# EPFL-VILAB/MultiMAE

Hardware: NVIDIA H100
Metric: MultiMAE-B pretrain samples/sec @ bs=128/GPU (higher is better)
Workload: dtype bf16

## Files before the change

multimae_b200/csrc/common.cuh:

```cuda
#pragma once

#include <cuda.h>
#include <cuda_bf16.h>
#include <cuda_runtime.h>
#include <stdint.h>

namespace mmae {

typedef __nv_bfloat16 bf16;

void set_last_error(const char* fmt, ...);

#define MMAE_CHECK(cond, code, ...)                    \
  do {                                                 \
    if (!(cond)) {                                     \
      ::mmae::set_last_error(__VA_ARGS__);             \
      return (code);                                   \
    }                                                  \
  } while (0)

#define MMAE_CUDA_OK(expr)                                                               \
  do {                                                                                   \
    cudaError_t _e = (expr);                                                             \
    if (_e != cudaSuccess) {                                                             \
// ... 129 lines not shown

__device__ __forceinline__ uint4 ld_stream_16_rw(const void* p) {
  uint4 v;
  asm volatile("ld.global.L1::no_allocate.v4.u32 {%0, %1, %2, %3}, [%4];"
               : "=r"(v.x), "=r"(v.y), "=r"(v.z), "=r"(v.w)
               : "l"(p));
  return v;
}

__device__ __forceinline__ void mbar_init(uint64_t* bar, uint32_t count) {
  asm volatile("mbarrier.init.shared::cta.b64 [%0], %1;" ::"r"(smem_u32(bar)), "r"(count) : "memory");
}
__device__ __forceinline__ void fence_barrier_init() {
  asm volatile("fence.mbarrier_init.release.cluster;" ::: "memory");
}
__device__ __forceinline__ void fence_proxy_async_smem() {
  asm volatile("fence.proxy.async.shared::cta;" ::: "memory");
}
__device__ __forceinline__ void mbar_expect_tx(uint64_t* bar, uint32_t bytes) {
  asm volatile("mbarrier.arrive.expect_tx.shared::cta.b64 _, [%0], %1;" ::"r"(smem_u32(bar)), "r"(bytes)
               : "memory");
}
__device__ __forceinline__ void mbar_arrive(uint64_t* bar) {
  asm volatile("mbarrier.arrive.shared::cta.b64 _, [%0];" ::"r"(smem_u32(bar)) : "memory");
}
__device__ __forceinline__ bool mbar_try_wait(uint64_t* bar, uint32_t parity) {
  uint32_t ok;
  asm volatile(
      "{\n\t"
      ".reg .pred P1;\n\t"
      "mbarrier.try_wait.parity.shared::cta.b64 P1, [%1], %2;\n\t"
      "selp.u32 %0, 1, 0, P1;\n\t"
      "}\n"
      : "=r"(ok)
      : "r"(smem_u32(bar)), "r"(parity)
      : "memory");
  return ok != 0;
}
__device__ __forceinline__ void mbar_wait(uint64_t* bar, uint32_t parity) {
  while (!mbar_try_wait(bar, parity)) {
  }
}

__device__ __forceinline__ void tma_prefetch_desc(const CUtensorMap* m) {
  asm volatile("prefetch.tensormap [%0];" ::"l"(reinterpret_cast<uint64_t>(m)) : "memory");
}
__device__ __forceinline__ void tma_load_2d(void* smem_dst, const CUtensorMap* m, uint64_t* bar, int c0,
                                            int c1) {
  asm volatile(
      "cp.async.bulk.tensor.2d.shared::cluster.global.mbarrier::complete_tx::bytes [%0], [%1, {%3, %4}], [%2];"
      :
      : "r"(smem_u32(smem_dst)), "l"(reinterpret_cast<uint64_t>(m)), "r"(smem_u32(bar)), "r"(c0), "r"(c1)
      : "memory");
}
__device__ __forceinline__ void tma_load_2d_multicast(void* smem_dst, const CUtensorMap* m, uint64_t* bar, int c0, int c1,
                                                      uint16_t cta_mask) {
  asm volatile(
      "cp.async.bulk.tensor.2d.shared::cluster.global.mbarrier::complete_tx::bytes.multicast::cluster [%0], [%1, {%3, %4}], "
      "[%2], %5;"
      :
      : "r"(smem_u32(smem_dst)), "l"(reinterpret_cast<uint64_t>(m)), "r"(smem_u32(bar)), "r"(c0), "r"(c1), "h"(cta_mask)
      : "memory");
}
__device__ __forceinline__ void tma_store_2d(const CUtensorMap* m, const void* smem_src, int c0, int c1) {
  asm volatile("cp.async.bulk.tensor.2d.global.shared::cta.bulk_group [%0, {%2, %3}], [%1];"
               :
               : "l"(reinterpret_cast<uint64_t>(m)), "r"(smem_u32(smem_src)), "r"(c0), "r"(c1)
               : "memory");
}
__device__ __forceinline__ void tma_reduce_add_2d(const CUtensorMap* m, const void* smem_src, int c0, int c1) {
  asm volatile("cp.reduce.async.bulk.tensor.2d.global.shared::cta.add.tile.bulk_group [%0, {%2, %3}], [%1];"
               :
               : "l"(reinterpret_cast<uint64_t>(m)), "r"(smem_u32(smem_src)), "r"(c0), "r"(c1)
               : "memory");
}
__device__ __forceinline__ void tma_store_3d(const CUtensorMap* m, const void* smem_src, int c0, int c1, int c2) {
  asm volatile("cp.async.bulk.tensor.3d.global.shared::cta.bulk_group [%0, {%2, %3, %4}], [%1];"
               :
               : "l"(reinterpret_cast<uint64_t>(m)), "r"(smem_u32(smem_src)), "r"(c0), "r"(c1), "r"(c2)
               : "memory");
}
__device__ __forceinline__ void bulk_commit_group() { asm volatile("cp.async.bulk.commit_group;" ::: "memory"); }
__device__ __forceinline__ void bulk_wait_read_all() { asm volatile("cp.async.bulk.wait_group.read 0;" ::: "memory"); }
__device__ __forceinline__ void bulk_wait_all() { asm volatile("cp.async.bulk.wait_group 0;" ::: "memory"); }
__device__ __forceinline__ void tma_load_3d(void* smem_dst, const CUtensorMap* m, uint64_t* bar, int c0,
                                            int c1, int c2) {
  asm volatile(
      "cp.async.bulk.tensor.3d.shared::cluster.global.mbarrier::complete_tx::bytes [%0], [%1, {%3, %4, %5}], "
      "[%2];"
      :
      : "r"(smem_u32(smem_dst)), "l"(reinterpret_cast<uint64_t>(m)), "r"(smem_u32(bar)), "r"(c0), "r"(c1),
        "r"(c2)
      : "memory");
}

__device__ __forceinline__ uint32_t cluster_ctarank() {
  uint32_t r;
  asm volatile("mov.u32 %0, %%cluster_ctarank;" : "=r"(r));
  return r;
}
__device__ __forceinline__ void cluster_sync_all() {
  asm volatile("barrier.cluster.arrive.release.aligned;\n\tbarrier.cluster.wait.acquire.aligned;" ::: "memory");
}
__device__ __forceinline__ uint32_t mapa_u32(uint32_t smem_addr, uint32_t rank) {
  uint32_t r;
  asm volatile("mapa.shared::cluster.u32 %0, %1, %2;" : "=r"(r) : "r"(smem_addr), "r"(rank));
  return r;
}

__device__ __forceinline__ void wgmma_fence() { asm volatile("wgmma.fence.sync.aligned;" ::: "memory"); }
__device__ __forceinline__ void wgmma_commit() { asm volatile("wgmma.commit_group.sync.aligned;" ::: "memory"); }
template <int N>
__device__ __forceinline__ void wgmma_wait() {
  asm volatile("wgmma.wait_group.sync.aligned %0;" ::"n"(N) : "memory");
}
__device__ __forceinline__ void reg_fence(float& r) { asm volatile("" : "+f"(r)::"memory"); }

template <int R>
__device__ __forceinline__ void setmaxnreg_inc() {
  asm volatile("setmaxnreg.inc.sync.aligned.u32 %0;" ::"n"(R));
}
template <int R>
__device__ __forceinline__ void setmaxnreg_dec() {
  asm volatile("setmaxnreg.dec.sync.aligned.u32 %0;" ::"n"(R));
}

__device__ __forceinline__ uint64_t gmma_desc_sw128(uint32_t smem_addr, uint32_t lbo_bytes, uint32_t sbo_bytes) {
  uint64_t d = 0;
  d |= uint64_t((smem_addr & 0x3FFFFu) >> 4);
  d |= uint64_t((lbo_bytes >> 4) & 0x3FFFu) << 16;
  d |= uint64_t((sbo_bytes >> 4) & 0x3FFFu) << 32;
  d |= uint64_t(1) << 62;
  return d;
}

__device__ __forceinline__ void mbar_arrive_cluster(uint32_t mbar_cluster) {
  asm volatile("mbarrier.arrive.release.cluster.shared::cluster.b64 _, [%0];" ::"r"(mbar_cluster) : "memory");
}

__device__ __forceinline__ uint64_t gmma_desc_noswz(uint32_t smem_addr, uint32_t lbo_bytes, uint32_t sbo_bytes) {
  uint64_t d = 0;
  d |= uint64_t((smem_addr & 0x3FFFFu) >> 4);
  d |= uint64_t((lbo_bytes >> 4) & 0x3FFFu) << 16;
  d |= uint64_t((sbo_bytes >> 4) & 0x3FFFu) << 32;
  return d;
}

template <int TA, int TB>
__device__ __forceinline__ void wgmma_m64n64k16(float (&d)[32], uint64_t desc_a, uint64_t desc_b, uint32_t scale_d) {
  asm volatile(
      "{\n.reg .pred p;\nsetp.ne.b32 p, %34, 0;\n"
      "wgmma.mma_async.sync.aligned.m64n64k16.f32.bf16.bf16 "
      "{"
      "%0, %1, %2, %3, %4, %5, %6, %7, %8, %9, %10, %11, %12, %13, %14, %15, "
      "%16, %17, %18, %19, %20, %21, %22, %23, %24, %25, %26, %27, %28, %29, %30, %31"
      "}, %32, %33, p, 1, 1, %35, %36;\n}\n"
      : "+f"(d[0]), "+f"(d[1]), "+f"(d[2]), "+f"(d[3]), "+f"(d[4]), "+f"(d[5]), "+f"(d[6]), "+f"(d[7]),
        "+f"(d[8]), "+f"(d[9]), "+f"(d[10]), "+f"(d[11]), "+f"(d[12]), "+f"(d[13]), "+f"(d[14]), "+f"(d[15]),
        "+f"(d[16]), "+f"(d[17]), "+f"(d[18]), "+f"(d[19]), "+f"(d[20]), "+f"(d[21]), "+f"(d[22]), "+f"(d[23]),
        "+f"(d[24]), "+f"(d[25]), "+f"(d[26]), "+f"(d[27]), "+f"(d[28]), "+f"(d[29]), "+f"(d[30]), "+f"(d[31])
      : "l"(desc_a), "l"(desc_b), "r"(scale_d), "n"(TA), "n"(TB));
}
template <int TA, int TB>
__device__ __forceinline__ void wgmma_m64n192k16(float (&d)[96], uint64_t desc_a, uint64_t desc_b, uint32_t scale_d) {
  asm volatile(
      "{\n.reg .pred p;\nsetp.ne.b32 p, %98, 0;\n"
// ... 117 lines not shown
```

multimae_b200/csrc/gemm_wgmma.cu:

```cuda
#include <algorithm>
#include <cstdlib>

#include "common.cuh"
#include "../../include/multimae_b200.h"

namespace mmae {

void count_launch();
bool gemm_profile_begin(cudaStream_t st, double flops, int M, int N, int K, int flags);
void gemm_profile_end(cudaStream_t st);

namespace {

constexpr int BM = 128;
constexpr int BK = 64;
constexpr int WG_K = 16;
constexpr int GEMM_THREADS = 384;

struct GemmParams {
  int M, N, K;
  int num_kb;
  int kb_per_split;
  int tma_store;
  mmae_gemm_epilogue ep;
};

template <int BN>
struct GemmCfg {
  static constexpr int STAGES = BN == 256 ? 4 : (BN == 192 ? 5 : (BN == 128 ? 6 : 8));
  static constexpr int A_BYTES = BM * BK * 2;
  static constexpr int B_BYTES = BN * BK * 2;
  static constexpr int STAGE_BYTES = A_BYTES + B_BYTES;
  static constexpr int BAR_OFFSET = STAGES * STAGE_BYTES;
  static constexpr int TOTAL = BAR_OFFSET + 256 + 1024;
  static_assert(TOTAL <= 232448, "GEMM exceeds the 227 KB shared-memory limit");
};

__device__ __forceinline__ void red_add_v2(float* addr, float a, float b) {
  asm volatile("red.global.add.v2.f32 [%0], {%1, %2};" ::"l"(addr), "f"(a), "f"(b) : "memory");
}

__device__ __forceinline__ void epilogue_pair(float v0, float v1, int row, int n, const GemmParams& p, bool first_split,
                                              bool atomic_out) {
  const mmae_gemm_epilogue& ep = p.ep;
  v0 *= ep.alpha;
  v1 *= ep.alpha;
  if (ep.bias && first_split) {
    const float2 b = __ldg(reinterpret_cast<const float2*>(ep.bias + n));
    v0 += b.x;
    v1 += b.y;
  }
  if (ep.preact_bf16)
    *reinterpret_cast<uint32_t*>(reinterpret_cast<bf16*>(ep.preact_bf16) + int64_t(row) * ep.ld_preact + n) = pack_bf16x2(v0, v1);
  if (ep.act == 1) {
    v0 = gelu_erf(v0);
    v1 = gelu_erf(v1);
  }
  if (ep.dgelu_z) {
    const uint32_t z = __ldg(reinterpret_cast<const unsigned int*>(reinterpret_cast<const bf16*>(ep.dgelu_z) +
                                                                   int64_t(row) * ep.ld_dgelu_z + n));
    const float2 zf = unpack_bf16x2(z);
    v0 *= dgelu_erf(zf.x);
    v1 *= dgelu_erf(zf.y);
  }
  if (ep.residual && first_split) {
    const float2 r = __ldg(reinterpret_cast<const float2*>(ep.residual + int64_t(row) * ep.ld_residual + n));
    v0 += r.x;
    v1 += r.y;
  }
  if (ep.out_f32) {
    float* dst = ep.out_f32 + int64_t(row) * ep.ld_out_f32 + n;
    if (atomic_out) red_add_v2(dst, v0, v1);
    else *reinterpret_cast<float2*>(dst) = make_float2(v0, v1);
  }
  if (ep.out_bf16)
    *reinterpret_cast<uint32_t*>(reinterpret_cast<bf16*>(ep.out_bf16) + int64_t(row) * ep.ld_out_bf16 + n) = pack_bf16x2(v0, v1);
}

template <typename T>
__device__ __forceinline__ void stage_pair(uint8_t* stage, int r, int c, float v0, float v1) {
  T* box = reinterpret_cast<T*>(stage + (c >> 5) * (64 * 32 * sizeof(T)));
  if constexpr (sizeof(T) == 4) *reinterpret_cast<float2*>(box + r * 32 + (c & 31)) = make_float2(v0, v1);
  else *reinterpret_cast<uint32_t*>(box + r * 32 + (c & 31)) = pack_bf16x2(v0, v1);
}

template <int BN, int CL, bool A_MN, bool B_MN>
__global__ void __launch_bounds__(GEMM_THREADS, 1)
    gemm_bf16_kernel(const __grid_constant__ CUtensorMap tmA, const __grid_constant__ CUtensorMap tmB,
                     const __grid_constant__ CUtensorMap tmC, const GemmParams p) {
  pdl_launch_dependents();
  using C = GemmCfg<BN>;
  constexpr int STAGES = C::STAGES;
  constexpr int BH = BN / CL;
  static_assert(!B_MN || BH % 64 == 0, "MN-major B is loaded in 64-column chunks");

  extern __shared__ uint8_t smem_raw[];
  const uint32_t raw_addr = smem_u32(smem_raw);
  uint8_t* smem = smem_raw + ((1024u - (raw_addr & 1023u)) & 1023u);
  uint64_t* full_bar = reinterpret_cast<uint64_t*>(smem + C::BAR_OFFSET);
  uint64_t* empty_bar = full_bar + STAGES;

  const int wg = threadIdx.x >> 7;
  const int rank = CL > 1 ? int(cluster_ctarank()) : 0;
  const int n0 = blockIdx.x * BN;
  const int m0 = blockIdx.y * BM;
  const int kb_begin = blockIdx.z * p.kb_per_split;
  int nkb = p.num_kb - kb_begin;
  if (nkb > p.kb_per_split) nkb = p.kb_per_split;
  if (nkb < 0) nkb = 0;

  if (threadIdx.x == 0) {
    tma_prefetch_desc(&tmA);
    tma_prefetch_desc(&tmB);
    if (p.tma_store) tma_prefetch_desc(&tmC);
#pragma unroll
    for (int s = 0; s < STAGES; ++s) {
      mbar_init(&full_bar[s], 1);
      mbar_init(&empty_bar[s], 2 * CL);
    }
    fence_barrier_init();
  }
  __syncthreads();
  if constexpr (CL > 1) cluster_sync_all();
  pdl_wait();

  if (wg == 0) {
    setmaxnreg_dec<40>();
    if (threadIdx.x == 0) {
      for (int kb = 0; kb < nkb; ++kb) {
        const int s = kb % STAGES;
        const uint32_t ph = (kb / STAGES) & 1;
        mbar_wait(&empty_bar[s], ph ^ 1u);
        mbar_expect_tx(&full_bar[s], C::STAGE_BYTES);
        uint8_t* sA = smem + s * C::STAGE_BYTES;
        uint8_t* sB = sA + C::A_BYTES;
        const int k0 = (kb_begin + kb) * BK;
        if constexpr (!A_MN) {
          tma_load_2d(sA, &tmA, &full_bar[s], k0, m0);
        } else {
#pragma unroll
          for (int c = 0; c < BM / 64; ++c) tma_load_2d(sA + c * (64 * BK * 2), &tmA, &full_bar[s], m0 + c * 64, k0);
        }
        if constexpr (CL == 1) {
          if constexpr (!B_MN) {
            tma_load_2d(sB, &tmB, &full_bar[s], k0, n0);
          } else {
#pragma unroll
            for (int c = 0; c < BN / 64; ++c) tma_load_2d(sB + c * (64 * BK * 2), &tmB, &full_bar[s], n0 + c * 64, k0);
          }
        } else {
          if constexpr (!B_MN) {
            tma_load_2d_multicast(sB + rank * BH * 128, &tmB, &full_bar[s], k0, n0 + rank * BH, 0x3);
          } else {
#pragma unroll
            for (int c = 0; c < BH / 64; ++c)
              tma_load_2d_multicast(sB + (rank * (BH / 64) + c) * (64 * BK * 2), &tmB, &full_bar[s], n0 + rank * BH + c * 64,
                                    k0, 0x3);
          }
        }
      }
    }
  } else {
    setmaxnreg_inc<232>();
    const int cw = wg - 1;
    float acc[BN / 2];

    for (int kb = 0; kb < nkb; ++kb) {
      const int s = kb % STAGES;
      const uint32_t ph = (kb / STAGES) & 1;
      mbar_wait(&full_bar[s], ph);
      const uint32_t a_addr = smem_u32(smem + s * C::STAGE_BYTES) + cw * (64 * BK * 2);
      const uint32_t b_addr = smem_u32(smem + s * C::STAGE_BYTES) + C::A_BYTES;
#pragma unroll
      for (int i = 0; i < BN / 2; ++i) reg_fence(acc[i]);
      wgmma_fence();
#pragma unroll
      for (int j = 0; j < BK / WG_K; ++j) {
        const uint32_t sd = (kb | j) != 0 ? 1u : 0u;
        const uint64_t da = A_MN ? gmma_desc_sw128(a_addr + j * (WG_K * 128), 64 * BK * 2, 1024)
                                 : gmma_desc_sw128(a_addr + j * (WG_K * 2), 16, 1024);
        const uint64_t db = B_MN ? gmma_desc_sw128(b_addr + j * (WG_K * 128), 64 * BK * 2, 1024)
                                 : gmma_desc_sw128(b_addr + j * (WG_K * 2), 16, 1024);
        if constexpr (BN == 256) wgmma_m64n256k16<A_MN ? 1 : 0, B_MN ? 1 : 0>(acc, da, db, sd);
        else if constexpr (BN == 192) wgmma_m64n192k16<A_MN ? 1 : 0, B_MN ? 1 : 0>(acc, da, db, sd);
        else if constexpr (BN == 128) wgmma_m64n128k16<A_MN ? 1 : 0, B_MN ? 1 : 0>(acc, da, db, sd);
        else wgmma_m64n64k16<A_MN ? 1 : 0, B_MN ? 1 : 0>(acc, da, db, sd);
      }
      wgmma_commit();
#pragma unroll
      for (int i = 0; i < BN / 2; ++i) reg_fence(acc[i]);
      wgmma_wait<1>();
      if (kb > 0 && (threadIdx.x & 127) == 0) {
        const int rs = (kb - 1) % STAGES;
        if constexpr (CL == 1) mbar_arrive(&empty_bar[rs]);
        else
          for (int r = 0; r < CL; ++r) mbar_arrive_cluster(mapa_u32(smem_u32(&empty_bar[rs]), uint32_t(r)));
      }
    }
    wgmma_wait<0>();
#pragma unroll
    for (int i = 0; i < BN / 2; ++i) reg_fence(acc[i]);

    const int t = threadIdx.x & 127;
    const int rl = (t >> 5) * 16 + ((t & 31) >> 2);
    const int row_a = m0 + cw * 64 + rl;
    const int row_b = row_a + 8;
    const bool first_split = blockIdx.z == 0;
    if (nkb > 0 && p.tma_store) {
      asm volatile("bar.sync 1, 256;" ::: "memory");
      uint8_t* stage = smem + cw * (64 * BN * (p.tma_store == 1 ? 2 : 4));
      const float* bias = first_split ? p.ep.bias : nullptr;
#pragma unroll
      for (int j = 0; j < BN / 8; ++j) {
        const int c = j * 8 + 2 * (t & 3);
        float v[4] = {acc[4 * j] * p.ep.alpha, acc[4 * j + 1] * p.ep.alpha, acc[4 * j + 2] * p.ep.alpha,
                      acc[4 * j + 3] * p.ep.alpha};
        if (bias && n0 + c < p.N) {
          const float2 bb = __ldg(reinterpret_cast<const float2*>(bias + n0 + c));
          v[0] += bb.x; v[1] += bb.y; v[2] += bb.x; v[3] += bb.y;
        }
        if (p.ep.act == 1) {
#pragma unroll
          for (int i = 0; i < 4; ++i) v[i] = gelu_erf(v[i]);
        }
        if (p.tma_store == 1) {
          stage_pair<bf16>(stage, rl, c, v[0], v[1]);
          stage_pair<bf16>(stage, rl + 8, c, v[2], v[3]);
        } else {
          stage_pair<float>(stage, rl, c, v[0], v[1]);
          stage_pair<float>(stage, rl + 8, c, v[2], v[3]);
        }
      }
      fence_proxy_async_smem();
      asm volatile("bar.sync %0, 128;" ::"r"(2 + cw) : "memory");
      if (t == 0) {
        const int box_bytes = 64 * 32 * (p.tma_store == 1 ? 2 : 4);
        for (int b = 0; b < BN / 32 && n0 + b * 32 < p.N; ++b) {
          if (p.tma_store == 3) tma_reduce_add_2d(&tmC, stage + b * box_bytes, n0 + b * 32, m0 + cw * 64);
          else tma_store_2d(&tmC, stage + b * box_bytes, n0 + b * 32, m0 + cw * 64);
        }
        bulk_commit_group();
        bulk_wait_all();
      }
    } else if (nkb > 0) {
      const bool atomic_out = p.ep.accumulate != 0 || gridDim.z > 1;
#pragma unroll
      for (int j = 0; j < BN / 8; ++j) {
        if (n0 + j * 8 >= p.N) break;
        const int n = n0 + j * 8 + 2 * (t & 3);
        if (row_a < p.M) epilogue_pair(acc[4 * j], acc[4 * j + 1], row_a, n, p, first_split, atomic_out);
        if (row_b < p.M) epilogue_pair(acc[4 * j + 2], acc[4 * j + 3], row_b, n, p, first_split, atomic_out);
      }
    }
  }
  if constexpr (CL > 1) cluster_sync_all();
}

template <int BN, int CL, bool A_MN, bool B_MN>
int launch_gemm(const CUtensorMap& tmA, const CUtensorMap& tmB, const CUtensorMap& tmC, const GemmParams& p, int split_k,
                cudaStream_t stream) {
  using C = GemmCfg<BN>;
  auto kern = gemm_bf16_kernel<BN, CL, A_MN, B_MN>;
  static bool configured = false;
  if (!configured) {
    MMAE_CUDA_OK(cudaFuncSetAttribute(kern, cudaFuncAttributeMaxDynamicSharedMemorySize, C::TOTAL));
    configured = true;
  }
  dim3 grid(ceil_div(p.N, BN), ceil_div(ceil_div(p.M, BM), CL) * CL, split_k);
  const bool prof = gemm_profile_begin(stream, 2.0 * p.M * p.N * p.K, p.M, p.N, p.K, (A_MN ? 1 : 0) | (B_MN ? 2 : 0) | (split_k << 8));
  if constexpr (CL == 1) {
    launch_k(kern, grid, GEMM_THREADS, C::TOTAL, stream, tmA, tmB, tmC, p);
  } else {
    cudaLaunchConfig_t cfg;
    memset(&cfg, 0, sizeof(cfg));
    cfg.gridDim = grid;
    cfg.blockDim = dim3(GEMM_THREADS);
    cfg.dynamicSmemBytes = C::TOTAL;
    cfg.stream = stream;
    cudaLaunchAttribute attr[2];
    attr[0].id = cudaLaunchAttributeClusterDimension;
    attr[0].val.clusterDim.x = 1;
    attr[0].val.clusterDim.y = CL;
    attr[0].val.clusterDim.z = 1;
    attr[1].id = cudaLaunchAttributeProgrammaticStreamSerialization;
    attr[1].val.programmaticStreamSerializationAllowed = 1;
    cfg.attrs = attr;
    cfg.numAttrs = pdl_enabled() ? 2 : 1;
    MMAE_CUDA_OK(cudaLaunchKernelEx(&cfg, kern, tmA, tmB, tmC, p));
  }
  if (prof) gemm_profile_end(stream);
  count_launch();
  MMAE_LAUNCH_OK();
  return MMAE_OK;
}

}
}

using namespace mmae;

static int g_gemm_variant = []() {
  const char* e = getenv("MMAE_GEMM_VARIANT");
  const int v = e ? atoi(e) : -1;
  return v >= -1 && v <= 6 ? v : -1;
}();
static int g_gemm_tma_store = []() {
  const char* e = getenv("MMAE_GEMM_TMA_STORE");
  return e ? (atoi(e) != 0) : 1;
}();

extern "C" int mmae_gemm_set_variant(int variant) {
  MMAE_CHECK(variant >= -1 && variant <= 6, MMAE_ERR_ARG, "mmae_gemm_set_variant: %d (-1 .. 6)", variant);
  g_gemm_variant = variant;
  return MMAE_OK;
}

extern "C" int mmae_gemm_set_tma_store(int enable) {
  g_gemm_tma_store = enable != 0;
  return MMAE_OK;
}

static int variant_bn(int v) { return v == 0 ? 64 : (v == 1 || v == 6) ? 128 : (v == 3 || v == 5) ? 192 : 256; }

extern "C" int mmae_gemm_bf16(const void* A, int64_t lda, int a_mn_major, const void* B, int64_t ldb,
                              int b_mn_major, int M, int N, int K, int split_k, const mmae_gemm_epilogue* ep,
                              void* stream) {
  MMAE_CHECK(A && B && ep, MMAE_ERR_ARG, "mmae_gemm_bf16: null operand");
  MMAE_CHECK(M > 0 && N > 0 && K > 0, MMAE_ERR_ARG, "mmae_gemm_bf16: bad shape M=%d N=%d K=%d", M, N, K);
  MMAE_CHECK(N % 8 == 0, MMAE_ERR_ARG, "mmae_gemm_bf16: N=%d must be a multiple of 8", N);
  MMAE_CHECK(lda % 8 == 0 && ldb % 8 == 0, MMAE_ERR_ARG, "mmae_gemm_bf16: lda/ldb must be multiples of 8");
  MMAE_CHECK((reinterpret_cast<uintptr_t>(A) & 15) == 0 && (reinterpret_cast<uintptr_t>(B) & 15) == 0,
             MMAE_ERR_ARG, "mmae_gemm_bf16: operands must be 16-byte aligned");
  MMAE_CHECK(ep->out_f32 || ep->out_bf16, MMAE_ERR_ARG, "mmae_gemm_bf16: no output");
  const int num_kb = ceil_div(K, BK);
  int variant = g_gemm_variant;
  const int sms = sm_count();
  const int tm = ceil_div(M, BM);
  if (split_k <= 0 && !(ep->out_f32 && !ep->out_bf16 && !ep->preact_bf16 && !ep->dgelu_z && ep->act == 0)) split_k = 1;
  if (split_k <= 0) {
    const int cand_var[2] = {1, 2};
    long best_cost = -1;
    int best_split = 1, best_var = variant >= 0 ? variant : 1;
    for (int i = 0; i < (variant >= 0 ? 1 : 2); ++i) {
      const int v = variant >= 0 ? variant : cand_var[i];
      const int bn = variant_bn(v);
      if (variant < 0 && bn > 128 && N < bn) continue;
      const int tiles = tm * ceil_div(N, bn);
      int s_ = std::max(1, sms / tiles);
      s_ = std::min(s_, std::max(1, num_kb / 4));
      const int kbps = ceil_div(num_kb, s_);
      s_ = ceil_div(num_kb, kbps);
      const long rounds = (long(tiles) * s_ + sms - 1) / sms;
      const long cost = rounds * bn * (kbps + 6);
      if (best_cost < 0 || cost < best_cost) {
        best_cost = cost;
        best_split = s_;
        best_var = v;
      }
    }
    split_k = best_split;
    variant = best_var;
  }
  if (split_k > num_kb) split_k = num_kb;
  const int kb_per_split = ceil_div(num_kb, split_k);
  split_k = ceil_div(num_kb, kb_per_split);
  if (split_k > 1 || ep->accumulate) {
    MMAE_CHECK(ep->out_f32 && !ep->out_bf16 && !ep->preact_bf16 && !ep->dgelu_z && ep->act == 0, MMAE_ERR_ARG,
               "mmae_gemm_bf16: split-K / accumulate supports only a linear fp32 epilogue");
  }
#define MMAE_LD_OK(ptr, ld) (!(ptr) || ((ld) % 8 == 0 && (reinterpret_cast<uintptr_t>(ptr) & 15) == 0))
  MMAE_CHECK(MMAE_LD_OK(ep->residual, ep->ld_residual) && MMAE_LD_OK(ep->dgelu_z, ep->ld_dgelu_z) &&
                 MMAE_LD_OK(ep->preact_bf16, ep->ld_preact) && MMAE_LD_OK(ep->out_f32, ep->ld_out_f32) &&
                 MMAE_LD_OK(ep->out_bf16, ep->ld_out_bf16) &&
                 (!ep->bias || (reinterpret_cast<uintptr_t>(ep->bias) & 15) == 0),
             MMAE_ERR_ARG, "mmae_gemm_bf16: epilogue tensors need 16-byte alignment and ld %% 8 == 0");
#undef MMAE_LD_OK

  if (variant < 0) {
    const int cand_var[2] = {1, 2};
    long best_cost = -1;
    variant = 1;
    for (int i = 0; i < 2; ++i) {
      const int bn = variant_bn(cand_var[i]);
      if (bn > 128 && N < bn) continue;
      const long items = long(tm) * ceil_div(N, bn) * split_k;
      const long rounds = (items + sms - 1) / sms;
      const long cost = rounds * (bn + 40);
      if (best_cost < 0 || cost < best_cost) {
        best_cost = cost;
        variant = cand_var[i];
      }
    }
  }
  if (variant == 5 && b_mn_major) variant = 4;
  const int BNsel = variant_bn(variant);
  const int CLsel = variant >= 4 ? 2 : 1;

  CUtensorMap tmA, tmB;
  int rc;
  if (!a_mn_major) {
    rc = make_tmap_2d_bf16(&tmA, A, (uint64_t)M, (uint64_t)K, (uint64_t)lda, BK, BM);
  } else {
    MMAE_CHECK(M % 8 == 0, MMAE_ERR_ARG, "mmae_gemm_bf16: MN-major A needs M %% 8 == 0");
    rc = make_tmap_2d_bf16(&tmA, A, (uint64_t)K, (uint64_t)M, (uint64_t)lda, 64, BK);
  }
  if (rc) return rc;
  if (!b_mn_major) {
    rc = make_tmap_2d_bf16(&tmB, B, (uint64_t)N, (uint64_t)K, (uint64_t)ldb, BK, BNsel / CLsel);
  } else {
    rc = make_tmap_2d_bf16(&tmB, B, (uint64_t)K, (uint64_t)N, (uint64_t)ldb, 64, BK);
  }
  if (rc) return rc;

  GemmParams p;
  p.M = M; p.N = N; p.K = K;
  p.num_kb = num_kb;
  p.kb_per_split = kb_per_split;
  p.ep = *ep;
  p.tma_store = 0;
  CUtensorMap tmC = tmA;
  if (g_gemm_tma_store && !ep->preact_bf16 && !ep->dgelu_z && !ep->residual) {
    if (ep->out_bf16 && !ep->out_f32 && split_k == 1 && !ep->accumulate) {
      p.tma_store = 1;
      rc = make_tmap_2d_store(&tmC, ep->out_bf16, 2, (uint64_t)M, (uint64_t)N, (uint64_t)ep->ld_out_bf16);
      if (rc) return rc;
    } else if (ep->out_f32 && !ep->out_bf16 && ep->act == 0) {
      p.tma_store = (split_k > 1 || ep->accumulate) ? 3 : 2;
      rc = make_tmap_2d_store(&tmC, ep->out_f32, 4, (uint64_t)M, (uint64_t)N, (uint64_t)ep->ld_out_f32);
      if (rc) return rc;
    }
  }
  cudaStream_t st = reinterpret_cast<cudaStream_t>(stream);
#define MMAE_DISPATCH(BN_, CL_)                                                                               \
  do {                                                                                                        \
    if (!a_mn_major && !b_mn_major) return launch_gemm<BN_, CL_, false, false>(tmA, tmB, tmC, p, split_k, st); \
    if (!a_mn_major && b_mn_major) return launch_gemm<BN_, CL_, false, true>(tmA, tmB, tmC, p, split_k, st);   \
    if (a_mn_major && !b_mn_major) return launch_gemm<BN_, CL_, true, false>(tmA, tmB, tmC, p, split_k, st);   \
    return launch_gemm<BN_, CL_, true, true>(tmA, tmB, tmC, p, split_k, st);                                  \
  } while (0)
  if (variant == 4) MMAE_DISPATCH(256, 2);
  if (variant == 6) MMAE_DISPATCH(128, 2);
  if (variant == 5) {
    if (!a_mn_major) return launch_gemm<192, 2, false, false>(tmA, tmB, tmC, p, split_k, st);
    return launch_gemm<192, 2, true, false>(tmA, tmB, tmC, p, split_k, st);
  }
  if (variant == 0) MMAE_DISPATCH(64, 1);
  if (variant == 3) MMAE_DISPATCH(192, 1);
  if (variant == 2) MMAE_DISPATCH(256, 1);
  MMAE_DISPATCH(128, 1);
#undef MMAE_DISPATCH
}
```

Measured before the change: 2935.

## Make the WGMMA GEMM persistent with pipelined TMA-store epilogue and joint split/tile selection

Turns the GEMM into a persistent kernel. Each CTA (or cluster) walks a strided list of work items, and the smem pipeline stage and phase counter keep running across tiles, so the producer can prefetch the next tile's operands while consumers do the current epilogue. The TMA-store epilogue now stages 32-column boxes through a small double- or quad-buffered region and waits only on older bulk groups, which overlaps stores with the staging of later boxes. The split-K and tile-variant heuristics are merged into one cost search, and BN=192 drops to 4 stages to make room for the epilogue buffers. The trade-offs are fewer pipeline stages for BN=192, more complex index decoding, and the risk of a launch-bound regression for small grids.

Result: faster. 3096, median of 6 (+5.5%).

```diff
diff --git a/multimae_b200/csrc/common.cuh b/multimae_b200/csrc/common.cuh
--- a/multimae_b200/csrc/common.cuh
+++ b/multimae_b200/csrc/common.cuh
@@ -235,6 +235,8 @@
 }
 __device__ __forceinline__ void bulk_commit_group() { asm volatile("cp.async.bulk.commit_group;" ::: "memory"); }
 __device__ __forceinline__ void bulk_wait_read_all() { asm volatile("cp.async.bulk.wait_group.read 0;" ::: "memory"); }
+template <int N>
+__device__ __forceinline__ void bulk_wait_read() { asm volatile("cp.async.bulk.wait_group.read %0;" ::"n"(N) : "memory"); }
 __device__ __forceinline__ void bulk_wait_all() { asm volatile("cp.async.bulk.wait_group 0;" ::: "memory"); }
 __device__ __forceinline__ void tma_load_3d(void* smem_dst, const CUtensorMap* m, uint64_t* bar, int c0,
                                             int c1, int c2) {
diff --git a/multimae_b200/csrc/gemm_wgmma.cu b/multimae_b200/csrc/gemm_wgmma.cu
--- a/multimae_b200/csrc/gemm_wgmma.cu
+++ b/multimae_b200/csrc/gemm_wgmma.cu
@@ -21,20 +21,41 @@
   int M, N, K;
   int num_kb;
   int kb_per_split;
+  int tiles_n;
+  int tiles_m;
+  int splits;
   int tma_store;
   mmae_gemm_epilogue ep;
 };
 
 template <int BN>
 struct GemmCfg {
-  static constexpr int STAGES = BN == 256 ? 4 : (BN == 192 ? 5 : (BN == 128 ? 6 : 8));
+  static constexpr int STAGES = BN == 256 ? 4 : (BN == 192 ? 4 : (BN == 128 ? 6 : 8));
   static constexpr int A_BYTES = BM * BK * 2;
   static constexpr int B_BYTES = BN * BK * 2;
   static constexpr int STAGE_BYTES = A_BYTES + B_BYTES;
-  static constexpr int BAR_OFFSET = STAGES * STAGE_BYTES;
+  static constexpr int EPI_BOX_BYTES = 64 * 32 * 4;
+  static constexpr int EPI_OFFSET = STAGES * STAGE_BYTES;
+  static constexpr int BAR_OFFSET = EPI_OFFSET + 2 * 2 * EPI_BOX_BYTES;
   static constexpr int TOTAL = BAR_OFFSET + 256 + 1024;
   static_assert(TOTAL <= 232448, "GEMM exceeds the 227 KB shared-memory limit");
 };
+
+struct WorkItem {
+  int m0, n0, split, kb_begin, nkb;
+};
+
+template <int BN, int CL>
+__device__ __forceinline__ WorkItem decode_item(int item, const GemmParams& p, int rank) {
+  WorkItem w;
+  const int rest = item / p.tiles_n;
+  w.n0 = (item - rest * p.tiles_n) * BN;
+  w.split = rest / p.tiles_m;
+  w.m0 = ((rest - w.split * p.tiles_m) * CL + rank) * BM;
+  w.kb_begin = w.split * p.kb_per_split;
+  w.nkb = min(p.kb_per_split, p.num_kb - w.kb_begin);
+  return w;
+}
 
 __device__ __forceinline__ void red_add_v2(float* addr, float a, float b) {
   asm volatile("red.global.add.v2.f32 [%0], {%1, %2};" ::"l"(addr), "f"(a), "f"(b) : "memory");
@@ -78,10 +99,10 @@
 }
 
 template <typename T>
-__device__ __forceinline__ void stage_pair(uint8_t* stage, int r, int c, float v0, float v1) {
-  T* box = reinterpret_cast<T*>(stage + (c >> 5) * (64 * 32 * sizeof(T)));
-  if constexpr (sizeof(T) == 4) *reinterpret_cast<float2*>(box + r * 32 + (c & 31)) = make_float2(v0, v1);
-  else *reinterpret_cast<uint32_t*>(box + r * 32 + (c & 31)) = pack_bf16x2(v0, v1);
+__device__ __forceinline__ void stage_pair(uint8_t* box, int r, int c, float v0, float v1) {
+  T* b = reinterpret_cast<T*>(box);
+  if constexpr (sizeof(T) == 4) *reinterpret_cast<float2*>(b + r * 32 + c) = make_float2(v0, v1);
+  else *reinterpret_cast<uint32_t*>(b + r * 32 + c) = pack_bf16x2(v0, v1);
 }
 
 template <int BN, int CL, bool A_MN, bool B_MN>
@@ -102,12 +123,9 @@
 
   const int wg = threadIdx.x >> 7;
   const int rank = CL > 1 ? int(cluster_ctarank()) : 0;
-  const int n0 = blockIdx.x * BN;
-  const int m0 = blockIdx.y * BM;
-  const int kb_begin = blockIdx.z * p.kb_per_split;
-  int nkb = p.num_kb - kb_begin;
-  if (nkb > p.kb_per_split) nkb = p.kb_per_split;
-  if (nkb < 0) nkb = 0;
+  const int num_items = p.tiles_n * p.tiles_m * p.splits;
+  const int first_item = blockIdx.x / CL;
+  const int item_stride = gridDim.x / CL;
 
   if (threadIdx.x == 0) {
     tma_prefetch_desc(&tmA);
@@ -127,35 +145,39 @@
   if (wg == 0) {
     setmaxnreg_dec<40>();
     if (threadIdx.x == 0) {
-      for (int kb = 0; kb < nkb; ++kb) {
-        const int s = kb % STAGES;
-        const uint32_t ph = (kb / STAGES) & 1;
-        mbar_wait(&empty_bar[s], ph ^ 1u);
-        mbar_expect_tx(&full_bar[s], C::STAGE_BYTES);
-        uint8_t* sA = smem + s * C::STAGE_BYTES;
-        uint8_t* sB = sA + C::A_BYTES;
-        const int k0 = (kb_begin + kb) * BK;
-        if constexpr (!A_MN) {
-          tma_load_2d(sA, &tmA, &full_bar[s], k0, m0);
-        } else {
-#pragma unroll
-          for (int c = 0; c < BM / 64; ++c) tma_load_2d(sA + c * (64 * BK * 2), &tmA, &full_bar[s], m0 + c * 64, k0);
-        }
-        if constexpr (CL == 1) {
-          if constexpr (!B_MN) {
-            tma_load_2d(sB, &tmB, &full_bar[s], k0, n0);
+      uint32_t it = 0;
+      for (int item = first_item; item < num_items; item += item_stride) {
+        const WorkItem w = decode_item<BN, CL>(item, p, rank);
+        for (int kb = 0; kb < w.nkb; ++kb, ++it) {
+          const int s = it % STAGES;
+          const uint32_t ph = (it / STAGES) & 1;
+          mbar_wait(&empty_bar[s], ph ^ 1u);
+          mbar_expect_tx(&full_bar[s], C::STAGE_BYTES);
+          uint8_t* sA = smem + s * C::STAGE_BYTES;
+          uint8_t* sB = sA + C::A_BYTES;
+          const int k0 = (w.kb_begin + kb) * BK;
+          if constexpr (!A_MN) {
+            tma_load_2d(sA, &tmA, &full_bar[s], k0, w.m0);
           } else {
 #pragma unroll
-            for (int c = 0; c < BN / 64; ++c) tma_load_2d(sB + c * (64 * BK * 2), &tmB, &full_bar[s], n0 + c * 64, k0);
+            for (int c = 0; c < BM / 64; ++c) tma_load_2d(sA + c * (64 * BK * 2), &tmA, &full_bar[s], w.m0 + c * 64, k0);
           }
-        } else {
-          if constexpr (!B_MN) {
-            tma_load_2d_multicast(sB + rank * BH * 128, &tmB, &full_bar[s], k0, n0 + rank * BH, 0x3);
+          if constexpr (CL == 1) {
+            if constexpr (!B_MN) {
+              tma_load_2d(sB, &tmB, &full_bar[s], k0, w.n0);
+            } else {
+#pragma unroll
+              for (int c = 0; c < BN / 64; ++c) tma_load_2d(sB + c * (64 * BK * 2), &tmB, &full_bar[s], w.n0 + c * 64, k0);
+            }
           } else {
-#pragma unroll
-            for (int c = 0; c < BH / 64; ++c)
-              tma_load_2d_multicast(sB + (rank * (BH / 64) + c) * (64 * BK * 2), &tmB, &full_bar[s], n0 + rank * BH + c * 64,
-                                    k0, 0x3);
+            if constexpr (!B_MN) {
+              tma_load_2d_multicast(sB + rank * BH * 128, &tmB, &full_bar[s], k0, w.n0 + rank * BH, 0x3);
+            } else {
+#pragma unroll
+              for (int c = 0; c < BH / 64; ++c)
+                tma_load_2d_multicast(sB + (rank * (BH / 64) + c) * (64 * BK * 2), &tmB, &full_bar[s],
+                                      w.n0 + rank * BH + c * 64, k0, 0x3);
+            }
           }
         }
       }
@@ -163,131 +185,161 @@
   } else {
     setmaxnreg_inc<232>();
     const int cw = wg - 1;
-    float acc[BN / 2];
-
-    for (int kb = 0; kb < nkb; ++kb) {
-      const int s = kb % STAGES;
-      const uint32_t ph = (kb / STAGES) & 1;
-      mbar_wait(&full_bar[s], ph);
-      const uint32_t a_addr = smem_u32(smem + s * C::STAGE_BYTES) + cw * (64 * BK * 2);
-      const uint32_t b_addr = smem_u32(smem + s * C::STAGE_BYTES) + C::A_BYTES;
-#pragma unroll
-      for (int i = 0; i < BN / 2; ++i) reg_fence(acc[i]);
-      wgmma_fence();
-#pragma unroll
-      for (int j = 0; j < BK / WG_K; ++j) {
-        const uint32_t sd = (kb | j) != 0 ? 1u : 0u;
-        const uint64_t da = A_MN ? gmma_desc_sw128(a_addr + j * (WG_K * 128), 64 * BK * 2, 1024)
-                                 : gmma_desc_sw128(a_addr + j * (WG_K * 2), 16, 1024);
-        const uint64_t db = B_MN ? gmma_desc_sw128(b_addr + j * (WG_K * 128), 64 * BK * 2, 1024)
-                                 : gmma_desc_sw128(b_addr + j * (WG_K * 2), 16, 1024);
-        if constexpr (BN == 256) wgmma_m64n256k16<A_MN ? 1 : 0, B_MN ? 1 : 0>(acc, da, db, sd);
-        else if constexpr (BN == 192) wgmma_m64n192k16<A_MN ? 1 : 0, B_MN ? 1 : 0>(acc, da, db, sd);
-        else if constexpr (BN == 128) wgmma_m64n128k16<A_MN ? 1 : 0, B_MN ? 1 : 0>(acc, da, db, sd);
-        else wgmma_m64n64k16<A_MN ? 1 : 0, B_MN ? 1 : 0>(acc, da, db, sd);
-      }
-      wgmma_commit();
-#pragma unroll
-      for (int i = 0; i < BN / 2; ++i) reg_fence(acc[i]);
-      wgmma_wait<1>();
-      if (kb > 0 && (threadIdx.x & 127) == 0) {
-        const int rs = (kb - 1) % STAGES;
-        if constexpr (CL == 1) mbar_arrive(&empty_bar[rs]);
-        else
-          for (int r = 0; r < CL; ++r) mbar_arrive_cluster(mapa_u32(smem_u32(&empty_bar[rs]), uint32_t(r)));
-      }
-    }
-    wgmma_wait<0>();
-#pragma unroll
-    for (int i = 0; i < BN / 2; ++i) reg_fence(acc[i]);
-
     const int t = threadIdx.x & 127;
     const int rl = (t >> 5) * 16 + ((t & 31) >> 2);
-    const int row_a = m0 + cw * 64 + rl;
-    const int row_b = row_a + 8;
-    const bool first_split = blockIdx.z == 0;
-    if (nkb > 0 && p.tma_store) {
-      asm volatile("bar.sync 1, 256;" ::: "memory");
-      uint8_t* stage = smem + cw * (64 * BN * (p.tma_store == 1 ? 2 : 4));
-      const float* bias = first_split ? p.ep.bias : nullptr;
-#pragma unroll
-      for (int j = 0; j < BN / 8; ++j) {
-        const int c = j * 8 + 2 * (t & 3);
-        float v[4] = {acc[4 * j] * p.ep.alpha, acc[4 * j + 1] * p.ep.alpha, acc[4 * j + 2] * p.ep.alpha,
-                      acc[4 * j + 3] * p.ep.alpha};
-        if (bias && n0 + c < p.N) {
-          const float2 bb = __ldg(reinterpret_cast<const float2*>(bias + n0 + c));
-          v[0] += bb.x; v[1] += bb.y; v[2] += bb.x; v[3] += bb.y;
+    uint8_t* epi = smem + C::EPI_OFFSET + cw * (2 * C::EPI_BOX_BYTES);
+    const bool atomic_out = p.ep.accumulate != 0 || p.splits > 1;
+    uint32_t it = 0;
+    uint32_t boxes = 0;
+    auto release = [&](int s) {
+      if (t == 0) {
+        if constexpr (CL == 1) mbar_arrive(&empty_bar[s]);
+        else
+          for (int r = 0; r < CL; ++r) mbar_arrive_cluster(mapa_u32(smem_u32(&empty_bar[s]), uint32_t(r)));
+      }
+    };
+    float acc[BN / 2];
+
+    for (int item = first_item; item < num_items; item += item_stride) {
+      const WorkItem w = decode_item<BN, CL>(item, p, rank);
+      for (int kb = 0; kb < w.nkb; ++kb, ++it) {
+        const int s = it % STAGES;
+        const uint32_t ph = (it / STAGES) & 1;
+        mbar_wait(&full_bar[s], ph);
+        const uint32_t a_addr = smem_u32(smem + s * C::STAGE_BYTES) + cw * (64 * BK * 2);
+        const uint32_t b_addr = smem_u32(smem + s * C::STAGE_BYTES) + C::A_BYTES;
+#pragma unroll
+        for (int i = 0; i < BN / 2; ++i) reg_fence(acc[i]);
+        wgmma_fence();
+#pragma unroll
+        for (int j = 0; j < BK / WG_K; ++j) {
+          const uint32_t sd = (kb | j) != 0 ? 1u : 0u;
+          const uint64_t da = A_MN ? gmma_desc_sw128(a_addr + j * (WG_K * 128), 64 * BK * 2, 1024)
+                                   : gmma_desc_sw128(a_addr + j * (WG_K * 2), 16, 1024);
+          const uint64_t db = B_MN ? gmma_desc_sw128(b_addr + j * (WG_K * 128), 64 * BK * 2, 1024)
+                                   : gmma_desc_sw128(b_addr + j * (WG_K * 2), 16, 1024);
+          if constexpr (BN == 256) wgmma_m64n256k16<A_MN ? 1 : 0, B_MN ? 1 : 0>(acc, da, db, sd);
+          else if constexpr (BN == 192) wgmma_m64n192k16<A_MN ? 1 : 0, B_MN ? 1 : 0>(acc, da, db, sd);
+          else if constexpr (BN == 128) wgmma_m64n128k16<A_MN ? 1 : 0, B_MN ? 1 : 0>(acc, da, db, sd);
+          else wgmma_m64n64k16<A_MN ? 1 : 0, B_MN ? 1 : 0>(acc, da, db, sd);
         }
-        if (p.ep.act == 1) {
-#pragma unroll
-          for (int i = 0; i < 4; ++i) v[i] = gelu_erf(v[i]);
+        wgmma_commit();
+#pragma unroll
+        for (int i = 0; i < BN / 2; ++i) reg_fence(acc[i]);
+        wgmma_wait<1>();
+        if (kb > 0) release((it - 1) % STAGES);
+      }
+      wgmma_wait<0>();
+#pragma unroll
+      for (int i = 0; i < BN / 2; ++i) reg_fence(acc[i]);
+      release((it - 1) % STAGES);
+
+      const int row_a = w.m0 + cw * 64 + rl;
+      const int row_b = row_a + 8;
+      const bool first_split = w.split == 0;
+      if (p.tma_store) {
+        const float* bias = first_split ? p.ep.bias : nullptr;
+        const bool bf16_out = p.tma_store == 1;
+#pragma unroll
+        for (int b = 0; b < BN / 32; ++b) {
+          if (w.n0 + b * 32 >= p.N) break;
+          uint8_t* box = bf16_out ? epi + (boxes & 3) * (C::EPI_BOX_BYTES / 2) : epi + (boxes & 1) * C::EPI_BOX_BYTES;
+          if (t == 0) {
+            if (bf16_out) bulk_wait_read<3>();
+            else bulk_wait_read<1>();
+          }
+          asm volatile("bar.sync %0, 128;" ::"r"(2 + cw) : "memory");
+#pragma unroll
+          for (int jj = 0; jj < 4; ++jj) {
+            const int j = 4 * b + jj;
+            const int c = jj * 8 + 2 * (t & 3);
+            float v[4] = {acc[4 * j] * p.ep.alpha, acc[4 * j + 1] * p.ep.alpha, acc[4 * j + 2] * p.ep.alpha,
+                          acc[4 * j + 3] * p.ep.alpha};
+            if (bias && w.n0 + b * 32 + c < p.N) {
+              const float2 bb = __ldg(reinterpret_cast<const float2*>(bias + w.n0 + b * 32 + c));
+              v[0] += bb.x; v[1] += bb.y; v[2] += bb.x; v[3] += bb.y;
+            }
+            if (p.ep.act == 1) {
+#pragma unroll
+              for (int i = 0; i < 4; ++i) v[i] = gelu_erf(v[i]);
+            }
+            if (bf16_out) {
+              stage_pair<bf16>(box, rl, c, v[0], v[1]);
+              stage_pair<bf16>(box, rl + 8, c, v[2], v[3]);
+            } else {
+              stage_pair<float>(box, rl, c, v[0], v[1]);
+              stage_pair<float>(box, rl + 8, c, v[2], v[3]);
+            }
+          }
+          fence_proxy_async_smem();
+          asm volatile("bar.sync %0, 128;" ::"r"(2 + cw) : "memory");
+          if (t == 0) {
+            if (p.tma_store == 3) tma_reduce_add_2d(&tmC, box, w.n0 + b * 32, w.m0 + cw * 64);
+            else tma_store_2d(&tmC, box, w.n0 + b * 32, w.m0 + cw * 64);
+            bulk_commit_group();
+          }
+          ++boxes;
         }
-        if (p.tma_store == 1) {
-          stage_pair<bf16>(stage, rl, c, v[0], v[1]);
-          stage_pair<bf16>(stage, rl + 8, c, v[2], v[3]);
-        } else {
-          stage_pair<float>(stage, rl, c, v[0], v[1]);
-          stage_pair<float>(stage, rl + 8, c, v[2], v[3]);
+      } else {
+#pragma unroll
+        for (int j = 0; j < BN / 8; ++j) {
+          if (w.n0 + j * 8 >= p.N) break;
+          const int n = w.n0 + j * 8 + 2 * (t & 3);
+          if (row_a < p.M) epilogue_pair(acc[4 * j], acc[4 * j + 1], row_a, n, p, first_split, atomic_out);
+          if (row_b < p.M) epilogue_pair(acc[4 * j + 2], acc[4 * j + 3], row_b, n, p, first_split, atomic_out);
         }
       }
-      fence_proxy_async_smem();
-      asm volatile("bar.sync %0, 128;" ::"r"(2 + cw) : "memory");
-      if (t == 0) {
-        const int box_bytes = 64 * 32 * (p.tma_store == 1 ? 2 : 4);
-        for (int b = 0; b < BN / 32 && n0 + b * 32 < p.N; ++b) {
-          if (p.tma_store == 3) tma_reduce_add_2d(&tmC, stage + b * box_bytes, n0 + b * 32, m0 + cw * 64);
-          else tma_store_2d(&tmC, stage + b * box_bytes, n0 + b * 32, m0 + cw * 64);
-        }
-        bulk_commit_group();
-        bulk_wait_all();
-      }
-    } else if (nkb > 0) {
-      const bool atomic_out = p.ep.accumulate != 0 || gridDim.z > 1;
-#pragma unroll
-      for (int j = 0; j < BN / 8; ++j) {
-        if (n0 + j * 8 >= p.N) break;
-        const int n = n0 + j * 8 + 2 * (t & 3);
-        if (row_a < p.M) epilogue_pair(acc[4 * j], acc[4 * j + 1], row_a, n, p, first_split, atomic_out);
-        if (row_b < p.M) epilogue_pair(acc[4 * j + 2], acc[4 * j + 3], row_b, n, p, first_split, atomic_out);
-      }
-    }
+    }
+    if (t == 0 && p.tma_store) bulk_wait_all();
   }
   if constexpr (CL > 1) cluster_sync_all();
 }
 
 template <int BN, int CL, bool A_MN, bool B_MN>
-int launch_gemm(const CUtensorMap& tmA, const CUtensorMap& tmB, const CUtensorMap& tmC, const GemmParams& p, int split_k,
+int launch_gemm(const CUtensorMap& tmA, const CUtensorMap& tmB, const CUtensorMap& tmC, const GemmParams& p,
                 cudaStream_t stream) {
   using C = GemmCfg<BN>;
   auto kern = gemm_bf16_kernel<BN, CL, A_MN, B_MN>;
-  static bool configured = false;
-  if (!configured) {
+  cudaLaunchConfig_t cfg;
+  memset(&cfg, 0, sizeof(cfg));
+  cfg.blockDim = dim3(GEMM_THREADS);
+  cfg.dynamicSmemBytes = C::TOTAL;
+  cfg.stream = stream;
+  cudaLaunchAttribute attr[2];
+  attr[0].id = cudaLaunchAttributeClusterDimension;
+  attr[0].val.clusterDim.x = CL;
+  attr[0].val.clusterDim.y = 1;
+  attr[0].val.clusterDim.z = 1;
+  attr[1].id = cudaLaunchAttributeProgrammaticStreamSerialization;
+  attr[1].val.programmaticStreamSerializationAllowed = 1;
+  cfg.attrs = attr;
+  cfg.numAttrs = 1;
+  static int resident = 0;
+  if (resident == 0) {
     MMAE_CUDA_OK(cudaFuncSetAttribute(kern, cudaFuncAttributeMaxDynamicSharedMemorySize, C::TOTAL));
-    configured = true;
-  }
-  dim3 grid(ceil_div(p.N, BN), ceil_div(ceil_div(p.M, BM), CL) * CL, split_k);
-  const bool prof = gemm_profile_begin(stream, 2.0 * p.M * p.N * p.K, p.M, p.N, p.K, (A_MN ? 1 : 0) | (B_MN ? 2 : 0) | (split_k << 8));
+    if constexpr (CL > 1) {
+      cfg.gridDim = dim3(CL);
+      MMAE_CUDA_OK(cudaOccupancyMaxActiveClusters(&resident, kern, &cfg));
+    } else {
+      int dev = 0, sms = 0;
+      MMAE_CUDA_OK(cudaGetDevice(&dev));
+      MMAE_CUDA_OK(cudaDeviceGetAttribute(&sms, cudaDevAttrMultiProcessorCount, dev));
+      resident = sms;
+    }
+    MMAE_CHECK(resident > 0, MMAE_ERR_CUDA, "mmae_gemm_bf16: the GEMM kernel does not fit on an SM");
+  }
+  const int items = p.tiles_n * p.tiles_m * p.splits;
+  const int slots = std::min(resident, std::max(1, sm_count() / CL));
+  cfg.gridDim = dim3(std::min(items, slots) * CL);
+  const bool prof = gemm_profile_begin(stream, 2.0 * p.M * p.N * p.K, p.M, p.N, p.K,
+                                       (A_MN ? 1 : 0) | (B_MN ? 2 : 0) | (p.splits << 8));
   if constexpr (CL == 1) {
-    launch_k(kern, grid, GEMM_THREADS, C::TOTAL, stream, tmA, tmB, tmC, p);
+    cfg.attrs = attr + 1;
+    cfg.numAttrs = pdl_enabled() ? 1 : 0;
   } else {
-    cudaLaunchConfig_t cfg;
-    memset(&cfg, 0, sizeof(cfg));
-    cfg.gridDim = grid;
-    cfg.blockDim = dim3(GEMM_THREADS);
-    cfg.dynamicSmemBytes = C::TOTAL;
-    cfg.stream = stream;
-    cudaLaunchAttribute attr[2];
-    attr[0].id = cudaLaunchAttributeClusterDimension;
-    attr[0].val.clusterDim.x = 1;
-    attr[0].val.clusterDim.y = CL;
-    attr[0].val.clusterDim.z = 1;
-    attr[1].id = cudaLaunchAttributeProgrammaticStreamSerialization;
-    attr[1].val.programmaticStreamSerializationAllowed = 1;
-    cfg.attrs = attr;
     cfg.numAttrs = pdl_enabled() ? 2 : 1;
-    MMAE_CUDA_OK(cudaLaunchKernelEx(&cfg, kern, tmA, tmB, tmC, p));
-  }
+  }
+  MMAE_CUDA_OK(cudaLaunchKernelEx(&cfg, kern, tmA, tmB, tmC, p));
   if (prof) gemm_profile_end(stream);
   count_launch();
   MMAE_LAUNCH_OK();
@@ -321,6 +373,9 @@
 }
 
 static int variant_bn(int v) { return v == 0 ? 64 : (v == 1 || v == 6) ? 128 : (v == 3 || v == 5) ? 192 : 256; }
+
+constexpr int KB_PER_ITEM_FIXED = 4;
+constexpr int MIN_KB_PER_SPLIT = 16;
 
 extern "C" int mmae_gemm_bf16(const void* A, int64_t lda, int a_mn_major, const void* B, int64_t ldb,
                               int b_mn_major, int M, int N, int K, int split_k, const mmae_gemm_epilogue* ep,
@@ -333,29 +388,33 @@
              MMAE_ERR_ARG, "mmae_gemm_bf16: operands must be 16-byte aligned");
   MMAE_CHECK(ep->out_f32 || ep->out_bf16, MMAE_ERR_ARG, "mmae_gemm_bf16: no output");
   const int num_kb = ceil_div(K, BK);
-  int variant = g_gemm_variant;
   const int sms = sm_count();
   const int tm = ceil_div(M, BM);
   if (split_k <= 0 && !(ep->out_f32 && !ep->out_bf16 && !ep->preact_bf16 && !ep->dgelu_z && ep->act == 0)) split_k = 1;
-  if (split_k <= 0) {
+
+  int variant = g_gemm_variant;
+  {
     const int cand_var[2] = {1, 2};
+    const int nvar = variant >= 0 ? 1 : 2;
     long best_cost = -1;
     int best_split = 1, best_var = variant >= 0 ? variant : 1;
-    for (int i = 0; i < (variant >= 0 ? 1 : 2); ++i) {
+    for (int i = 0; i < nvar; ++i) {
       const int v = variant >= 0 ? variant : cand_var[i];
-      const int bn = variant_bn(v);
+      const int bn = variant_bn(v), cl = v >= 4 ? 2 : 1;
       if (variant < 0 && bn > 128 && N < bn) continue;
-      const int tiles = tm * ceil_div(N, bn);
-      int s_ = std::max(1, sms / tiles);
-      s_ = std::min(s_, std::max(1, num_kb / 4));
-      const int kbps = ceil_div(num_kb, s_);
-      s_ = ceil_div(num_kb, kbps);
-      const long rounds = (long(tiles) * s_ + sms - 1) / sms;
-      const long cost = rounds * bn * (kbps + 6);
-      if (best_cost < 0 || cost < best_cost) {
-        best_cost = cost;
-        best_split = s_;
-        best_var = v;
+      const long tiles = long(ceil_div(tm, cl)) * ceil_div(N, bn);
+      const int slots = std::max(1, sms / cl);
+      const int s_lo = split_k > 0 ? split_k : 1;
+      const int s_hi = split_k > 0 ? split_k : std::max(1, num_kb / MIN_KB_PER_SPLIT);
+      for (int s = s_lo; s <= s_hi; ++s) {
+        const int kbps = ceil_div(num_kb, std::min(s, num_kb));
+        const long rounds = (tiles * ceil_div(num_kb, kbps) + slots - 1) / slots;
+        const long cost = rounds * (bn + 40) * cl * (kbps + KB_PER_ITEM_FIXED);
+        if (best_cost < 0 || cost < best_cost) {
+          best_cost = cost;
+          best_split = s;
+          best_var = v;
+        }
       }
     }
     split_k = best_split;
@@ -376,22 +435,6 @@
              MMAE_ERR_ARG, "mmae_gemm_bf16: epilogue tensors need 16-byte alignment and ld %% 8 == 0");
 #undef MMAE_LD_OK
 
-  if (variant < 0) {
-    const int cand_var[2] = {1, 2};
-    long best_cost = -1;
-    variant = 1;
-    for (int i = 0; i < 2; ++i) {
-      const int bn = variant_bn(cand_var[i]);
-      if (bn > 128 && N < bn) continue;
-      const long items = long(tm) * ceil_div(N, bn) * split_k;
-      const long rounds = (items + sms - 1) / sms;
-      const long cost = rounds * (bn + 40);
-      if (best_cost < 0 || cost < best_cost) {
-        best_cost = cost;
-        variant = cand_var[i];
-      }
-    }
-  }
   if (variant == 5 && b_mn_major) variant = 4;
   const int BNsel = variant_bn(variant);
   const int CLsel = variant >= 4 ? 2 : 1;
@@ -416,6 +459,9 @@
   p.M = M; p.N = N; p.K = K;
   p.num_kb = num_kb;
   p.kb_per_split = kb_per_split;
+  p.tiles_n = ceil_div(N, BNsel);
+  p.tiles_m = ceil_div(tm, CLsel);
+  p.splits = split_k;
   p.ep = *ep;
   p.tma_store = 0;
   CUtensorMap tmC = tmA;
@@ -431,18 +477,18 @@
     }
   }
   cudaStream_t st = reinterpret_cast<cudaStream_t>(stream);
-#define MMAE_DISPATCH(BN_, CL_)                                                                               \
-  do {                                                                                                        \
-    if (!a_mn_major && !b_mn_major) return launch_gemm<BN_, CL_, false, false>(tmA, tmB, tmC, p, split_k, st); \
-    if (!a_mn_major && b_mn_major) return launch_gemm<BN_, CL_, false, true>(tmA, tmB, tmC, p, split_k, st);   \
-    if (a_mn_major && !b_mn_major) return launch_gemm<BN_, CL_, true, false>(tmA, tmB, tmC, p, split_k, st);   \
-    return launch_gemm<BN_, CL_, true, true>(tmA, tmB, tmC, p, split_k, st);                                  \
+#define MMAE_DISPATCH(BN_, CL_)                                                                      \
+  do {                                                                                               \
+    if (!a_mn_major && !b_mn_major) return launch_gemm<BN_, CL_, false, false>(tmA, tmB, tmC, p, st); \
+    if (!a_mn_major && b_mn_major) return launch_gemm<BN_, CL_, false, true>(tmA, tmB, tmC, p, st);   \
+    if (a_mn_major && !b_mn_major) return launch_gemm<BN_, CL_, true, false>(tmA, tmB, tmC, p, st);   \
+    return launch_gemm<BN_, CL_, true, true>(tmA, tmB, tmC, p, st);                                  \
   } while (0)
   if (variant == 4) MMAE_DISPATCH(256, 2);
   if (variant == 6) MMAE_DISPATCH(128, 2);
   if (variant == 5) {
-    if (!a_mn_major) return launch_gemm<192, 2, false, false>(tmA, tmB, tmC, p, split_k, st);
-    return launch_gemm<192, 2, true, false>(tmA, tmB, tmC, p, split_k, st);
+    if (!a_mn_major) return launch_gemm<192, 2, false, false>(tmA, tmB, tmC, p, st);
+    return launch_gemm<192, 2, true, false>(tmA, tmB, tmC, p, st);
   }
   if (variant == 0) MMAE_DISPATCH(64, 1);
   if (variant == 3) MMAE_DISPATCH(192, 1);
```
